# zhoubin-me/agent0

Measured on NVIDIA B200. Metric: replay_sample_target_transitions_per_sec, higher is better.
Workload: dtype u8 frames / f32 targets / f64 n-step returns

## Files before the change

### agent0_b200/_lib.py

```python
import ctypes as C
import os

import torch

_PKG = os.path.dirname(os.path.abspath(__file__))
LIB_PATH = os.environ.get("A0_LIB") or os.path.join(_PKG, "libagent0_b200.so")

A0_SLOTS = 8
A0_REC_META_I32 = 14
A0_MAX_NSTEP = 16
A0_MAX_ACTIONS = 32
A0_MAX_QUANTILES = 256
PTR_FRAMES, PTR_REC_SLOTS, PTR_REC_INFO, PTR_TREE, PTR_MAX_P = range(5)
OPT_PDL = 1
K2B_PLAN_MAX = 1024
K2B_PLAN_BYTES = 90176


def lz4_stride(frame_bytes):
    n = 8 * int(frame_bytes)
    return (n + n // 255 + 20 + 15) // 16 * 16

_vp, _i32, _i64, _f32, _f64 = C.c_void_p, C.c_int32, C.c_int64, C.c_float, C.c_double


class LossCommon(C.Structure):
    _fields_ = [("B", _i32), ("A", _i32), ("action", _vp), ("reward", _vp), ("done", _vp),
                ("weight", _vp), ("gamma_n", _f32), ("alpha", _f32), ("eps", _f32),
                ("loss", _vp), ("prio", _vp), ("max_p", _vp)]


class Plan(C.Structure):
    _fields_ = [("m", _i32), ("n_new", _i32), ("n_marks", _i32), ("new_frame_pos", C.POINTER(_i32)),
                ("rec_meta", C.POINTER(_i32)), ("marks", C.POINTER(_i32))]


class Merge(C.Structure):
    _fields_ = [("n_place", _i64), ("place", C.POINTER(_i64)), ("n_rec", _i64), ("record_map", C.POINTER(_i64)),
                ("n_tail", _i64), ("tails", C.POINTER(_i64)), ("stride_hint", _i64)]


IX_HEAD_Q, IX_TAIL_Q, IX_HEAD_FS, IX_TOP, IX_REC_CAPACITY, IX_FRAME_CAPACITY, IX_NSTEP, IX_AGE_LIMIT, \
    IX_MAX_CHUNK, IX_STATE_WORDS = range(10)
INGEST_FRAMES_ON_DEVICE, INGEST_FRAMES_PINNED, INGEST_COPY_STREAM = 1, 2, 4

SIGNATURES = {
    "a0_version": (_i32, []),
    "a0_last_error": (C.c_char_p, []),
    "a0_set_option": (_i32, [_i32, _i64]),
    "a0_get_option": (_i32, [_i32, C.POINTER(C.c_int64)]),
    "a0_rb_create": (_i32, [C.POINTER(_vp), _i64, _i64, _i32, _i32]),
    "a0_rb_destroy": (_i32, [_vp]),
    "a0_rb_reset": (_i32, [_vp, _vp]),
    "a0_rb_ptr": (_vp, [_vp, _i32]),
    "a0_rb_tree_leaves": (_i64, [_vp]),
    "a0_ix_create": (_i32, [C.POINTER(_vp), _i64, _i64, _i32, _i64]),
    "a0_ix_destroy": (_i32, [_vp]),
    "a0_ix_state": (_i32, [_vp, _vp]),
    "a0_ix_sampleable": (_vp, [_vp]),
    "a0_ix_set_stack": (_i32, [_vp, _i64, _vp]),
    "a0_ix_get_stack": (_i32, [_vp, _i64, _vp]),
    "a0_ix_resolve_shift": (_i32, [_vp, _vp, _vp, _i32, _vp]),
    "a0_ix_plan": (_i32, [_vp, _vp, _vp, _i32, _i32, _vp, _vp, _vp, C.POINTER(Plan)]),
    "a0_dd_create": (_i32, [C.POINTER(_vp), _i32]),
    "a0_dd_destroy": (_i32, [_vp]),
    "a0_dd_resolve": (_i32, [_vp, _vp, _vp, _vp, _i32, _vp, _vp, C.POINTER(_i32)]),
    "a0_ex_create": (_i32, [C.POINTER(_vp), _vp, _vp]),
    "a0_ex_destroy": (_i32, [_vp]),
    "a0_ex_extend": (_i32, [_vp, _vp, _vp, _vp, _vp, _vp, _vp, _i32, _f32, _vp]),
    "a0_ex_extend_v": (_i32, [_vp, _vp, _vp, _vp, _vp, _vp, _vp, _i32, _f32, _vp]),
    "a0_ex_decode": (_i32, [_vp, _vp, _vp, _i32, _vp, _vp, _vp]),
    "a0_ex_resolve": (_i32, [_vp, _vp, _vp, _i32, _vp, _vp, C.POINTER(_i32)]),
    "a0_ex_last_timing": (_i32, [_vp, _vp]),
    "a0_lz4_encode": (_i32, [_vp, _i32, _i32, _vp, _vp, _vp, _vp]),
    "a0_ix_serialize": (_i32, [_vp, _vp, _i64, C.POINTER(_i64)]),
    "a0_ix_deserialize": (_i32, [_vp, _vp, _i64]),
    "a0_ckpt_save": (_i32, [_vp, _vp, _vp, C.c_char_p, _vp, _i64, _vp]),
    "a0_ckpt_load": (_i32, [_vp, _vp, _vp, C.c_char_p, _vp, _i64, C.POINTER(_i64), _vp]),
    "a0_ckpt_last_timing": (_i32, [_vp]),
    "a0_ix_merge": (_i32, [_vp, _i32, _vp, _vp, _vp, _vp, _vp, _vp, _vp, _vp, _vp, _vp, _vp, C.POINTER(Merge)]),
    "a0_ckpt_info": (_i32, [C.c_char_p, _vp, _vp, _i64]),
    "a0_ckpt_merge": (_i32, [_vp, _vp, _vp, _vp, _i32, _vp, _vp, _vp, _vp, _i64, _vp, _vp]),
    "a0_rb_ingest_plan": (_i32, [_vp, C.POINTER(Plan), _vp, _vp, _i32, _f32, _vp]),
    "a0_rb_ingest_steps": (_i32, [_vp, _vp, _vp, _vp, _vp, _i32, _vp, _vp, _vp, _i32, _f32, _vp]),
    "a0_rb_ingest_steps_dyn": (_i32, [_vp, _vp, _vp, _vp, _vp, _i32, _vp, _vp, _vp, _i32, _f32, _f32, _i32, _vp]),
    "a0_rb_append": (_i32, [_vp, _vp, _vp, _i32, _vp, _i32, _vp]),
    "a0_pt_mark": (_i32, [_vp, _vp, _i32, _f32, _vp]),
    "a0_pt_update": (_i32, [_vp, _vp, _vp, _i32, _f32, _f32, _vp]),
    "a0_pt_update_report": (_i32, [_vp, _vp, _vp, _i32, _f32, _f32, _vp, _vp, _vp]),
    "a0_pt_update_overlapped": (_i32, [_vp, _vp, _vp, _i32, _f32, _f32, _vp, _vp, _vp]),
    "a0_pt_update_plan": (_i32, [_vp, _vp, _i32, _vp, _vp]),
    "a0_pt_update_apply": (_i32, [_vp, _vp, _vp, _i32, _f32, _f32, _vp, _vp, _vp, _vp]),
    "a0_host_map": (_i32, [_vp, C.POINTER(_vp)]),
    "a0_pt_set": (_i32, [_vp, _vp, _vp, _i32, _vp]),
    "a0_rb_set_dynamic": (_i32, [_vp, _f32, _f32, _f32, _vp]),
    "a0_pt_sample": (_i32, [_vp, _vp, _i32, _i32, _f32, _f32, _f32, _i32, _vp, _vp, _vp, _vp]),
    "a0_pt_sample_rng": (_i32, [_vp, C.c_uint64, _i64, _i32, _i32, _f32, _f32, _f32, _i32, _vp, _vp, _vp, _vp, _vp]),
    "a0_pt_rng_seek": (_i32, [_vp, C.c_uint64, _vp]),
    "a0_pt_sample_unique": (_i32, [_vp, C.c_uint64, _i64, _i32, _i32, _f32, _f32, _f32, _i32, _vp, _vp, _vp, _vp, _vp]),
    "a0_rb_gather": (_i32, [_vp, _vp, _i32, _i32, _f64, _vp, _vp, _vp, _vp, _vp, _vp, _vp, _i32, _vp]),
    "a0_rb_sample_gather": (_i32, [_vp, _vp, C.c_uint64, _i64, _i32, _i32, _f32, _f32, _f32, _i32, _vp, _vp, _vp, _i32, _f64,
                                   _vp, _vp, _vp, _vp, _vp, _vp, _vp, _vp]),
    "a0_rb_sample_mail": (_i32, [_vp, _vp, C.c_uint64, _i64, _i32, _i32, _f32, _f32, _f32, _i32, _vp, _vp, _vp, _vp]),
    "a0_rb_gather_mail": (_i32, [_vp, _i32, _i32, _i32, _i32, _f64, _vp, _vp, _vp, _vp, _vp, _vp, _vp, _vp]),
    "a0_rb_gather_unpaired": (_i32, [_vp, _i32, _vp, _vp]),
    "a0_rb_check_fault": (_i32, [_vp]),
    "a0_rb_gather_f32": (_i32, [_vp, _vp, _i32, _i32, _f64, _vp, _vp, _i32, _vp, _vp, _vp, _vp, _vp, _vp, _vp]),
    "a0_rb_gather_bf16": (_i32, [_vp, _vp, _i32, _i32, _f64, _vp, _vp, _i32, _vp, _vp, _vp, _vp, _vp, _vp, _vp]),
    "a0_loss_dqn": (_i32, [C.POINTER(LossCommon), _vp, _vp, _vp, _vp, _vp]),
    "a0_loss_mdqn": (_i32, [C.POINTER(LossCommon), _vp, _vp, _vp, _f32, _f32, _vp, _vp]),
    "a0_loss_c51": (_i32, [C.POINTER(LossCommon), _vp, _vp, _vp, _vp, _i32, _f32, _f32, _vp, _vp, _vp]),
    "a0_loss_quantile": (_i32, [C.POINTER(LossCommon), _i32, _vp, _vp, _vp, _vp, _i32, _i32, _vp,
                                _vp, _vp, _vp, _vp, _vp]),
    "a0_act_epsilon_greedy": (_i32, [_vp, _i32, _i32, _f64, _vp, _vp, _vp, _vp, _vp, _vp, _vp]),
    "a0_u8_to_f32": (_i32, [_vp, _vp, _i64, _i32, _vp]),
}

_lib = None


def load():
    global _lib
    if _lib is not None:
        return _lib
    if not os.path.exists(LIB_PATH):
        raise RuntimeError(
            f"{LIB_PATH} is missing: build it with `python -m agent0_b200.build` "
            "(agent0_b200 has no CPU fallback)")
    lib = C.CDLL(LIB_PATH)
    for name, (res, args) in SIGNATURES.items():
        fn = getattr(lib, name)
        fn.restype, fn.argtypes = res, args
    _lib = lib
    return lib


_pyingest = False


def pyingest():
    global _pyingest
    if _pyingest is False:
        path = os.path.join(_PKG, "_a0_pyingest.so")
        _pyingest = None
        if os.path.exists(path):
            try:
                h = C.PyDLL(path)
                h.a0_py_unpack.restype = _i64
                h.a0_py_unpack.argtypes = [C.py_object, _i64, _vp, _vp, _vp, _vp, _vp, _vp]
                h.a0_py_release.restype = None
                h.a0_py_release.argtypes = [_i64, _vp]
                h.a0_py_buffer_size.restype = _i64
                _pyingest = h
            except OSError:
                _pyingest = None
    return _pyingest


def check(rc, what):
    if rc != 0:
        msg = load().a0_last_error().decode(errors="replace")
        raise RuntimeError(f"{what} failed (code {rc}): {msg}")


_raw_stream = getattr(torch._C, "_cuda_getCurrentRawStream", None)


def stream_ptr(device=None):
    if _raw_stream is not None:
        if device is None:
            idx = torch.cuda.current_device()
        elif isinstance(device, int):
            idx = device
        else:
            idx = device.index if device.index is not None else torch.cuda.current_device()
        return _raw_stream(idx)
    return torch.cuda.current_stream(device).cuda_stream


def ptr(t, dtype=None):
    if t is None:
        return None
    if not t.is_cuda:
        raise RuntimeError("agent0_b200 kernels need CUDA tensors (there is no CPU path)")
    if dtype is not None and t.dtype != dtype:
        raise TypeError(f"expected {dtype}, got {t.dtype}")
    if not t.is_contiguous():
        raise ValueError("tensor must be contiguous")
    return t.data_ptr()


def host_map(t):
    if t.is_cuda or not t.is_pinned():
        raise ValueError("host_map needs a pinned CPU tensor")
    out = _vp()
    check(load().a0_host_map(t.data_ptr(), C.byref(out)), "a0_host_map")
    return out.value


class HandleOwner:

    def __init__(self, lib, handle):
        self.lib, self.handle = lib, handle

    def __del__(self):
        try:
            if self.handle is not None and self.handle.value:
                self.lib.a0_rb_destroy(self.handle)
                self.handle = None
        except Exception:
            pass


class _DevView:

    def __init__(self, address, shape, typestr, owner=None):
        self.owner = owner
        self.__cuda_array_interface__ = {"shape": tuple(shape), "typestr": typestr,
                                         "data": (int(address), False), "version": 2}


def device_view(address, shape, typestr, device, owner=None):
    return torch.as_tensor(_DevView(address, shape, typestr, owner), device=device)
```

### agent0_b200/csrc/a0_targets.cu

```cuda
#include <stdlib.h>

#include "a0_common.cuh"
#ifdef A0_TRACE
A0_TRACE_SETTER(a0_trace_set_targets)
#endif

struct A0Common {
  int32_t B, A;
  const int64_t* action;
  const float* reward;
  const float* done;
  const float* weight;
  float gamma_n, alpha, eps;
  float* loss;
  float* prio;
  float* max_p;
};

static inline A0Common a0_unpack(const a0_loss_common_t* c) {
  A0Common k;
  k.B = c->B; k.A = c->A; k.action = c->action; k.reward = c->reward; k.done = c->done;
  k.weight = c->weight; k.gamma_n = c->gamma_n; k.alpha = c->alpha; k.eps = c->eps;
  k.loss = c->loss; k.prio = c->prio; k.max_p = c->max_p;
  return k;
// ... 174 lines not shown
    if (!spec) l[k] = in ? orow[lane + 32 * k] : -INFINITY;
    s_m[wid][lane + 32 * k] = 0.0f;
  }
  if (spec) {
#pragma unroll
    for (int a2 = 0; a2 < C51_SPEC_A; ++a2)
      if (a2 == a) { l[0] = lo_all[a2][0]; l[1] = lo_all[a2][1]; }
  }

  float omx = -INFINITY;
#pragma unroll
  for (int k = 0; k < C51_MAXR; ++k) omx = fmaxf(omx, l[k]);
#ifdef A0_TRACE
  if (omx == 12345.678f) printf("x");
#endif
  A0_TX(0);
  int a_star;
  if (qsel) {
    float v = qs;
    int vi = lane;
#pragma unroll
    for (int o = 16; o > 0; o >>= 1) {
      const float ov = __shfl_xor_sync(0xffffffffu, v, o);
      const int oi = __shfl_xor_sync(0xffffffffu, vi, o);
      const float om = __shfl_xor_sync(0xffffffffu, omx, o);
      if (ov > v || (ov == v && oi < vi)) { v = ov; vi = oi; }
      omx = fmaxf(omx, om);
    }
    a_star = vi;
  } else {
    omx = a0_warp_max(omx);
    float best = -INFINITY;
    a_star = 0;
    for (int a2 = 0; a2 < A; ++a2) {
      const float* row = tgt_logits + ((size_t)b * A + a2) * M;
      float v[C51_MAXR], mx = -INFINITY;
#pragma unroll
      for (int k = 0; k < C51_MAXR; ++k) {
        v[k] = (k < R && lane + 32 * k < M) ? row[lane + 32 * k] : -INFINITY;
        mx = fmaxf(mx, v[k]);
      }
      mx = a0_warp_max(mx);
      float se = 0.0f;
#pragma unroll
      for (int k = 0; k < C51_MAXR; ++k) { v[k] = (k < R && lane + 32 * k < M) ? expf(v[k] - mx) : 0.0f; se += v[k]; }
      se = a0_warp_sum(se);
      float ev = 0.0f;
#pragma unroll
      for (int k = 0; k < C51_MAXR; ++k) ev += __fdiv_rn(v[k], se) * z[k];
      ev = a0_warp_sum(ev);
      if (ev > best) { best = ev; a_star = a2; }
    }
  }

  A0_TX(1);
  const float* trow = tgt_logits + ((size_t)b * A + a_star) * M;
  float p[C51_MAXR], mx = -INFINITY;
#pragma unroll
  for (int k = 0; k < C51_MAXR; ++k) p[k] = -INFINITY;
  if (spec) {
#pragma unroll
    for (int a2 = 0; a2 < C51_SPEC_A; ++a2)
      if (a2 == a_star) { p[0] = tg_all[a2][0]; p[1] = tg_all[a2][1]; }
  } else {
#pragma unroll
    for (int k = 0; k < C51_MAXR; ++k)
      if (k < R && lane + 32 * k < M) p[k] = trow[lane + 32 * k];
  }
#pragma unroll
  for (int k = 0; k < C51_MAXR; ++k) mx = fmaxf(mx, p[k]);
  float ose = 0.0f;
#pragma unroll
  for (int k = 0; k < C51_MAXR; ++k) ose += (k < R && lane + 32 * k < M) ? expf(l[k] - omx) : 0.0f;
#pragma unroll
  for (int o = 16; o > 0; o >>= 1) {
    const float om = __shfl_xor_sync(0xffffffffu, mx, o);
    const float os = __shfl_xor_sync(0xffffffffu, ose, o);
    mx = fmaxf(mx, om);
    ose += os;
  }
  float se = 0.0f;
#pragma unroll
  for (int k = 0; k < C51_MAXR; ++k) { p[k] = (k < R && lane + 32 * k < M) ? expf(p[k] - mx) : 0.0f; se += p[k]; }
  se = a0_warp_sum(se);

  A0_TX(2);
  const float gm = __fmul_rn(c.gamma_n, __fsub_rn(1.0f, d));
  const float delta = (vmax - vmin) / (float)(M - 1);
  int lo[C51_MAXR], up[C51_MAXR];
  float wlo[C51_MAXR], wup[C51_MAXR];
#pragma unroll
  for (int k = 0; k < C51_MAXR; ++k) {
    lo[k] = up[k] = -1;
    wlo[k] = wup[k] = 0.0f;
    if (k < R && lane + 32 * k < M) {
      const float pj = __fdiv_rn(p[k], se);
      float tz = __fadd_rn(r, __fmul_rn(gm, z[k]));
      tz = fminf(fmaxf(tz, vmin), vmax);
      const float base = __fdiv_rn(__fsub_rn(tz, vmin), delta);
      int lo_ = (int)floorf(base), up_ = (int)ceilf(base);
      if (up_ > 0 && lo_ == up_) lo_ -= 1;
      if (lo_ < M - 1 && lo_ == up_) up_ += 1;
      lo[k] = lo_; up[k] = up_ < M ? up_ : -1;
      wlo[k] = __fmul_rn(pj, __fsub_rn((float)up_, base));
      wup[k] = __fmul_rn(pj, __fsub_rn(base, (float)lo_));
    }
  }
  __syncwarp();
  A0_TX(3);
  if (R <= 2) {
    const int key4[4] = {lo[0], lo[1], up[0], up[1]};
    float val4[4] = {wlo[0], wlo[1], wup[0], wup[1]};
    a0_c51_scatter<4>(s_m[wid], key4, val4, lane);
  } else {
    a0_c51_scatter<C51_MAXR>(s_m[wid], lo, wlo, lane);
    a0_c51_scatter<C51_MAXR>(s_m[wid], up, wup, lane);
  }
  float m[C51_MAXR];
#pragma unroll
  for (int k = 0; k < C51_MAXR; ++k) m[k] = s_m[wid][lane + 32 * k];

  A0_TX(4);
  const float lse = logf(ose);
  float ce = 0.0f, msum = 0.0f;
#pragma unroll
  for (int k = 0; k < C51_MAXR; ++k)
    if (k < R && lane + 32 * k < M) { ce += m[k] * ((l[k] - omx) - lse); msum += m[k]; }
  ce = a0_warp_sum(ce);
  msum = a0_warp_sum(msum);
  A0_TX(5);
  float* grow = grad + (size_t)b * A * M;
  for (int a2 = 0; a2 < A; ++a2) {
    if (a2 == a) continue;
    for (int j = lane; j < M; j += 32) grow[(size_t)a2 * M + j] = 0.0f;
  }
#pragma unroll
  for (int k = 0; k < C51_MAXR; ++k) {
    const int j = lane + 32 * k;
    if (k < R && j < M) {
      const float sm = expf((l[k] - omx) - lse);
      grow[(size_t)a * M + j] = w * (sm * msum - m[k]);
      if (target_prob) target_prob[(size_t)b * M + j] = m[k];
    }
  }
  A0_TX(6);
  if (lane == 0) a0_emit(c, b, -ce);
  A0_TX(7);
#ifdef A0_TRACE
  _t2 = _t2 * 0 + (unsigned long long)_c0;
#endif
  if (threadIdx.x == 0) A0_TEND(4);
}

template <int WARPS>
__global__ void __launch_bounds__(WARPS * 32)
a0_k4_c51_fast(const A0Common c, const float* __restrict__ logits, const float* __restrict__ tgt_logits,
               const float* __restrict__ qsel, const float* __restrict__ atoms, int32_t M, float vmin, float vmax,
               float delta, float* __restrict__ grad, float* __restrict__ target_prob) {
  __shared__ float s_m[WARPS][72];
  A0_T0();
  A0_PDL_PROLOGUE();
  A0_TMID();
#ifdef A0_TRACE
  const long long _c0 = clock64();
#endif
  const int lane = threadIdx.x & 31;
  const int wid = threadIdx.x >> 5;
  const int b = blockIdx.x * WARPS + wid;
  if (b >= c.B) return;
  const int A = c.A;
  const bool in0 = lane < M, in1 = lane + 32 < M;
  float lo_all[C51_SPEC_A][2], tg_all[C51_SPEC_A][2], qs[C51_SPEC_A];
  const float* lrow = logits + (size_t)b * A * M + lane;
  const float* trow = tgt_logits + (size_t)b * A * M + lane;
  const float* qrow = qsel + (size_t)b * A;
#pragma unroll
  for (int a2 = 0; a2 < C51_SPEC_A; ++a2) {
    const bool on = a2 < A;
    lo_all[a2][0] = (on && in0) ? lrow[a2 * M] : -INFINITY;
    lo_all[a2][1] = (on && in1) ? lrow[a2 * M + 32] : -INFINITY;
    tg_all[a2][0] = (on && in0) ? trow[a2 * M] : -INFINITY;
    tg_all[a2][1] = (on && in1) ? trow[a2 * M + 32] : -INFINITY;
    qs[a2] = on ? qrow[a2] : -INFINITY;
  }
  const int a = (int)c.action[b];
  const float r = c.reward[b], d = c.done[b], w = c.weight[b];
  const float z0 = in0 ? atoms[lane] : 0.0f, z1 = in1 ? atoms[lane + 32] : 0.0f;
  s_m[wid][lane] = 0.0f;
  s_m[wid][lane + 32] = 0.0f;
  const int AM = A * M, r0 = a * M;
  float* gb = grad + (size_t)b * AM;
  for (int e = lane; e < AM; e += 32)
    if (e < r0 || e >= r0 + M) gb[e] = 0.0f;
  int a_star = 0;
  float best = qs[0];
#pragma unroll
  for (int a2 = 1; a2 < C51_SPEC_A; ++a2)
    if (qs[a2] > best) { best = qs[a2]; a_star = a2; }
  float l0 = -INFINITY, l1 = -INFINITY, p0 = -INFINITY, p1 = -INFINITY;
#pragma unroll
  for (int a2 = 0; a2 < C51_SPEC_A; ++a2) {
    if (a2 == a) { l0 = lo_all[a2][0]; l1 = lo_all[a2][1]; }
    if (a2 == a_star) { p0 = tg_all[a2][0]; p1 = tg_all[a2][1]; }
  }
  A0_TX(0);
  float omx = fmaxf(l0, l1), mx = fmaxf(p0, p1);
#pragma unroll
  for (int o = 16; o > 0; o >>= 1) {
    const float a_ = __shfl_xor_sync(0xffffffffu, omx, o);
    const float b_ = __shfl_xor_sync(0xffffffffu, mx, o);
    omx = fmaxf(omx, a_);
    mx = fmaxf(mx, b_);
  }
  A0_TX(1);
  const float eo0 = in0 ? expf(l0 - omx) : 0.0f, eo1 = in1 ? expf(l1 - omx) : 0.0f;
  p0 = in0 ? expf(p0 - mx) : 0.0f;
  p1 = in1 ? expf(p1 - mx) : 0.0f;
  float ose = eo0 + eo1, se = p0 + p1;
#pragma unroll
  for (int o = 16; o > 0; o >>= 1) {
    const float a_ = __shfl_xor_sync(0xffffffffu, ose, o);
    const float b_ = __shfl_xor_sync(0xffffffffu, se, o);
    ose += a_;
    se += b_;
  }
  A0_TX(2);
  const float gm = __fmul_rn(c.gamma_n, __fsub_rn(1.0f, d));
  int k0 = -1, k1 = -1;
  float wl0 = 0.0f, wu0 = 0.0f, wl1 = 0.0f, wu1 = 0.0f;
  {
    const float pj0 = p0 != 0.0f ? __fdiv_rn(p0, se) : 0.0f, pj1 = p1 != 0.0f ? __fdiv_rn(p1, se) : 0.0f;
    const float tz0 = fminf(fmaxf(__fadd_rn(r, __fmul_rn(gm, z0)), vmin), vmax);
    const float tz1 = fminf(fmaxf(__fadd_rn(r, __fmul_rn(gm, z1)), vmin), vmax);
    const float nu0 = __fsub_rn(tz0, vmin), nu1 = __fsub_rn(tz1, vmin);
    const float bs0 = nu0 != 0.0f ? __fdiv_rn(nu0, delta) : 0.0f, bs1 = nu1 != 0.0f ? __fdiv_rn(nu1, delta) : 0.0f;
    const int c0 = max((int)ceilf(bs0) - 1, 0), c1 = max((int)ceilf(bs1) - 1, 0);
    if (in0) { k0 = c0; wl0 = __fmul_rn(pj0, __fsub_rn((float)(c0 + 1), bs0)); wu0 = __fmul_rn(pj0, __fsub_rn(bs0, (float)c0)); }
    if (in1) { k1 = c1; wl1 = __fmul_rn(pj1, __fsub_rn((float)(c1 + 1), bs1)); wu1 = __fmul_rn(pj1, __fsub_rn(bs1, (float)c1)); }
  }
  A0_TX(3);
#pragma unroll
  for (int dd = 1; dd < 32; dd <<= 1) {
    const int q0 = __shfl_up_sync(0xffffffffu, k0, dd), q1 = __shfl_up_sync(0xffffffffu, k1, dd);
    const float a0_ = __shfl_up_sync(0xffffffffu, wl0, dd), b0_ = __shfl_up_sync(0xffffffffu, wu0, dd);
    const float a1_ = __shfl_up_sync(0xffffffffu, wl1, dd), b1_ = __shfl_up_sync(0xffffffffu, wu1, dd);
    if (lane >= dd && q0 == k0) { wl0 = __fadd_rn(wl0, a0_); wu0 = __fadd_rn(wu0, b0_); }
    if (lane >= dd && q1 == k1) { wl1 = __fadd_rn(wl1, a1_); wu1 = __fadd_rn(wu1, b1_); }
  }
  const int n0 = __shfl_down_sync(0xffffffffu, k0, 1), n1 = __shfl_down_sync(0xffffffffu, k1, 1);
  const bool tail0 = k0 >= 0 && (lane == 31 || n0 != k0), tail1 = k1 >= 0 && (lane == 31 || n1 != k1);
  float* bins = s_m[wid];
  __syncwarp();
  if (tail0) bins[k0] = __fadd_rn(bins[k0], wl0);
  __syncwarp();
  if (tail1) bins[k1] = __fadd_rn(bins[k1], wl1);
  __syncwarp();
  if (tail0) bins[k0 + 1] = __fadd_rn(bins[k0 + 1], wu0);
  __syncwarp();
  if (tail1) bins[k1 + 1] = __fadd_rn(bins[k1 + 1], wu1);
  __syncwarp();
  const float m0 = bins[lane], m1 = bins[lane + 32];
  A0_TX(4);
  const float lse = logf(ose);
  const float ls0 = (l0 - omx) - lse, ls1 = (l1 - omx) - lse;
  float ce = 0.0f, msum = 0.0f;
  if (in0) { ce += m0 * ls0; msum += m0; }
  if (in1) { ce += m1 * ls1; msum += m1; }
#pragma unroll
  for (int o = 16; o > 0; o >>= 1) {
    const float a_ = __shfl_xor_sync(0xffffffffu, ce, o);
    const float b_ = __shfl_xor_sync(0xffffffffu, msum, o);
    ce += a_;
    msum += b_;
  }
  A0_TX(5);
  if (lane == 0) a0_emit(c, b, -ce);
  const float g0 = w * (expf(ls0) * msum - m0), g1 = w * (expf(ls1) * msum - m1);
  if (in0) gb[r0 + lane] = g0;
  if (in1) gb[r0 + lane + 32] = g1;
  if (target_prob) {
    if (in0) target_prob[(size_t)b * M + lane] = m0;
    if (in1) target_prob[(size_t)b * M + lane + 32] = m1;
  }
  A0_TX(6);
  A0_TX(7);
#ifdef A0_TRACE
  _t2 = _t2 * 0 + (unsigned long long)_c0;
#endif
  if (threadIdx.x == 0) A0_TEND(4);
}

static int g_c51_fast = -1;
static bool a0_option_c51_fast() {
  if (g_c51_fast < 0) {
    const char* e = getenv("A0_C51_FAST");
    g_c51_fast = e ? (atoi(e) != 0) : 1;
  }
  return g_c51_fast != 0;
}
void a0_set_c51_fast(int on) { g_c51_fast = on != 0; }

extern "C" int a0_loss_c51(const a0_loss_common_t* c, const float* logits, const float* tgt_logits,
                           const float* qsel, const float* atoms, int32_t M, float vmin, float vmax, float* grad,
                           float* target_prob, a0_stream_t stream) {
  int rc = a0_check_common(c, "a0_loss_c51");
  if (rc) return rc;
  A0_REQUIRE(logits && tgt_logits && atoms && grad, "a0_loss_c51: NULL tensor");
  A0_REQUIRE(M >= 2 && M <= C51_MAXR * 32, "a0_loss_c51: num_atoms %d outside [2,%d]", M, C51_MAXR * 32);
  A0_REQUIRE(vmax > vmin, "a0_loss_c51: vmax must exceed vmin");
  if (c->B == 0) return A0_OK;
  if (qsel && c->A <= C51_SPEC_A && M <= 64 && a0_option_c51_fast()) {
    const float delta = (vmax - vmin) / (float)(M - 1);
    static int warps = 0;
    if (!warps) {
      const char* e = getenv("A0_C51_WARPS");
      warps = e ? atoi(e) : C51_FAST_WARPS;
      if (warps != 1 && warps != 2 && warps != 4 && warps != 8 && warps != 16 && warps != 32) warps = C51_FAST_WARPS;
    }
    const unsigned grid = (unsigned)((c->B + warps - 1) / warps);
#define A0_C51_FAST_LAUNCH(W)                                                                                              \
    A0_LAUNCH(a0_k4_c51_fast<W>, grid, W * 32, 0, (cudaStream_t)stream, 1, A0_PDL_K4, a0_unpack(c), logits, tgt_logits, qsel,   \
              atoms, M, vmin, vmax, delta, grad, target_prob)
    if (warps == 1) A0_C51_FAST_LAUNCH(1);
    else if (warps == 2) A0_C51_FAST_LAUNCH(2);
    else if (warps == 4) A0_C51_FAST_LAUNCH(4);
    else if (warps == 8) A0_C51_FAST_LAUNCH(8);
    else if (warps == 16) A0_C51_FAST_LAUNCH(16);
    else A0_C51_FAST_LAUNCH(32);
#undef A0_C51_FAST_LAUNCH
    return A0_OK;
  }
  A0_LAUNCH(a0_k4_c51, (unsigned)((c->B + C51_WARPS - 1) / C51_WARPS), C51_WARPS * 32, 0, (cudaStream_t)stream, 1, A0_PDL_K4,
            a0_unpack(c), logits, tgt_logits, qsel, atoms, M, vmin, vmax, grad, target_prob);
  return A0_OK;
}

constexpr int QH_SPEC_A = 8;

__device__ __forceinline__ float a0_block_sum(float v, float* red, int nwarps) {
  v = a0_warp_sum(v);
  __syncthreads();
  if ((threadIdx.x & 31) == 0) red[threadIdx.x >> 5] = v;
  __syncthreads();
  float s = 0.0f;
  for (int i = 0; i < nwarps; ++i) s += red[i];
  return s;
}

template <bool SPEC>
__global__ void __launch_bounds__(A0_MAX_QUANTILES)
a0_k4_quantile(const A0Common c, int32_t layout, const float* __restrict__ q, const float* __restrict__ qt,
               const float* __restrict__ taus, const float* __restrict__ qsel, int32_t Ni, int32_t Nj,
               float* __restrict__ grad, const float* __restrict__ q_bar, const float* __restrict__ taus_full,
               float* __restrict__ fraction_loss, float* __restrict__ grad_taus) {
  __shared__ float sT[A0_MAX_QUANTILES];
  __shared__ float sQ[A0_MAX_QUANTILES];
  __shared__ float sMean[A0_MAX_ACTIONS];
  __shared__ float red[A0_MAX_QUANTILES / 32];
  __shared__ int s_astar;
  A0_PDL_PROLOGUE();
  const int b = blockIdx.x;
  const int tid = threadIdx.x, lane = tid & 31, wid = tid >> 5;
  const int nwarps = blockDim.x >> 5;
  const int A = c.A;
  const size_t sN_q = layout == 0 ? 1 : (size_t)A, sA_q = layout == 0 ? (size_t)Nj : 1;
  const size_t sN_t = layout == 0 ? 1 : (size_t)A, sA_t = layout == 0 ? (size_t)Ni : 1;
  const float* qb = q + (size_t)b * A * Nj;
  const float* tb = qt + (size_t)b * A * Ni;

  float qj = 0.0f, tau = 0.0f, w;
  int a;
  if (SPEC) {
    a = (int)c.action[b];
    const float r = c.reward[b], d = c.done[b];
    w = c.weight[b];
    float qs[QH_SPEC_A], tv[QH_SPEC_A], qv[QH_SPEC_A];
#pragma unroll
    for (int a2 = 0; a2 < QH_SPEC_A; ++a2) {
      const bool on = a2 < A;
      qs[a2] = on ? qsel[(size_t)b * A + a2] : -INFINITY;
      tv[a2] = (on && tid < Ni) ? tb[(size_t)tid * A + a2] : 0.0f;
      qv[a2] = (on && tid < Nj) ? qb[(size_t)tid * A + a2] : 0.0f;
    }
    if (tid < Nj) tau = taus[(size_t)b * Nj + tid];
    int a_star = 0;
    float best = qs[0];
#pragma unroll
    for (int a2 = 1; a2 < QH_SPEC_A; ++a2)
      if (qs[a2] > best) { best = qs[a2]; a_star = a2; }
    float tsel = 0.0f;
#pragma unroll
    for (int a2 = 0; a2 < QH_SPEC_A; ++a2) {
      if (a2 == a_star) tsel = tv[a2];
      if (a2 == a) qj = qv[a2];
    }
    if (tid < Ni) sT[tid] = a0_td_target(r, d, c.gamma_n, tsel);
    if (tid < Nj) sQ[tid] = qj;
    __syncthreads();
  } else {
  if (qsel) {
    if (wid == 0) {
      const int as = a0_warp_argmax(lane < A ? qsel[(size_t)b * A + lane] : -INFINITY, lane);
      if (lane == 0) s_astar = as;
    }
  } else {
    for (int a2 = wid; a2 < A; a2 += nwarps) {
      float s = 0.0f;
      for (int i = lane; i < Ni; i += 32) s += tb[a2 * sA_t + i * sN_t];
      s = a0_warp_sum(s);
      if (lane == 0) sMean[a2] = __fdiv_rn(s, (float)Ni);
    }
    __syncthreads();
    if (wid == 0) {
      const int as = a0_warp_argmax(lane < A ? sMean[lane] : -INFINITY, lane);
      if (lane == 0) s_astar = as;
    }
  }
  __syncthreads();
  const int a_star = s_astar;
  a = (int)c.action[b];
  const float r = c.reward[b], d = c.done[b];
  w = c.weight[b];
  if (tid < Ni) sT[tid] = a0_td_target(r, d, c.gamma_n, tb[a_star * sA_t + tid * sN_t]);
  if (tid < Nj) {
    qj = qb[a * sA_q + tid * sN_q];
    tau = taus ? taus[(size_t)b * Nj + tid] : __fdiv_rn((float)(2 * tid + 1), 2.0f * (float)Nj);
    sQ[tid] = qj;
  }
  __syncthreads();
  }

  float lsum = 0.0f, gsum = 0.0f;
  if (tid < Nj) {
    float lp = 0.0f, ln = 0.0f, gp = 0.0f, gn = 0.0f;
#pragma unroll 8
    for (int i = 0; i < Ni; ++i) {
      const float uij = qj - sT[i];
      const float a_ = fabsf(uij);
      const float c_ = fminf(a_, 1.0f);
      const float x_ = fmaf(-0.5f, c_, a_);
      if (uij > 0.0f) { lp = fmaf(c_, x_, lp); gp += c_; }
      else { ln = fmaf(c_, x_, ln); gn += c_; }
    }
    const float k_pos = 1.0f - tau;
    lsum = fmaf(k_pos, lp, tau * ln);
    gsum = fmaf(k_pos, gp, -tau * gn);
  }
  const float total = a0_block_sum(lsum, red, nwarps);
  float* gb = grad + (size_t)b * A * Nj;
  for (int i = tid; i < A * Nj; i += blockDim.x) gb[i] = 0.0f;
  __syncthreads();
  if (tid < Nj) gb[a * sA_q + tid * sN_q] = __fdiv_rn(w, (float)Ni) * gsum;
  if (tid == 0) a0_emit(c, b, __fdiv_rn(total, (float)Ni));

  if (q_bar) {
    const int F = Nj;
    float gi = 0.0f, contrib = 0.0f;
    if (tid < F - 1) {
      const float* qbar_b = q_bar + (size_t)b * (F - 1) * A;
      const float qi = qbar_b[(size_t)tid * A + a];
      const float prev = tid == 0 ? sQ[0] : qbar_b[(size_t)(tid - 1) * A + a];
      const float next = tid == F - 2 ? sQ[F - 1] : qbar_b[(size_t)(tid + 1) * A + a];
      const float v1 = qi - sQ[tid], v2 = qi - sQ[tid + 1];
      gi = (qi > prev ? v1 : -v1) + (qi < next ? v2 : -v2);
      contrib = gi * taus_full[(size_t)b * (F + 1) + tid + 1];
    }
    const float fl = a0_block_sum(contrib, red, nwarps);
    if (tid == 0 && fraction_loss) fraction_loss[b] = fl;
    if (grad_taus) {
      float* gt = grad_taus + (size_t)b * (F + 1);
      if (tid < F - 1) gt[tid + 1] = w * gi;
      if (tid == 0) { gt[0] = 0.0f; gt[F] = 0.0f; }
    }
  }
}

constexpr int QS_MAX = A0_MAX_QUANTILES;
static_assert(QS_MAX == 256, "the merge tree below is written for 8 runs of 32");

__device__ __forceinline__ float a0_qs_next_up(float x) {
  const uint32_t b = __float_as_uint(x);
  if (x == 0.0f) return __uint_as_float(1u);
  return __uint_as_float((b >> 31) ? b - 1u : b + 1u);
}
__device__ __forceinline__ float a0_qs_pad(int idx) { return __uint_as_float(0x7f7fff00u + (uint32_t)idx); }

// ... 461 lines not shown
```

### include/agent0_b200.h

```cpp
#ifndef AGENT0_B200_H
#define AGENT0_B200_H

#include <stddef.h>
#include <stdint.h>

#ifdef __cplusplus
extern "C" {
#endif

typedef struct a0_replay a0_replay_t;
typedef struct a0_index a0_index_t;
typedef void* a0_stream_t;

#define A0_OK 0
#define A0_EINVAL (-1)
#define A0_ENOMEM (-2)
#define A0_EFAULT (-3)
#define A0_STACK 4
#define A0_SLOTS 8
#define A0_MAX_NSTEP 16
#define A0_MAX_ACTIONS 32
#define A0_MAX_QUANTILES 256
#define A0_REC_META_I32 14

// ... 57 lines not shown
int a0_dd_resolve(a0_dedupe_t* dd, a0_index_t* ix, const int64_t* stream, const uint8_t* frames,
                  int32_t m, int64_t* fs8_out, int64_t* new_src_out, int32_t* n_new_out);

typedef struct a0_extend a0_extend_t;
int a0_ex_create(a0_extend_t** out, a0_replay_t* h, a0_index_t* ix);
int a0_ex_destroy(a0_extend_t* ex);
int a0_ex_extend(a0_extend_t* ex, const uint8_t* blobs , const int64_t* blob_len ,
                 const int64_t* stream, const int64_t* action, const double* reward, const uint8_t* done,
                 int32_t m, float alpha, a0_stream_t cuda_stream);
int a0_ex_extend_v(a0_extend_t* ex, const uint8_t* const* blob_ptr ,
                   const int64_t* blob_len , const int64_t* stream, const int64_t* action,
                   const double* reward, const uint8_t* done, int32_t m, float alpha,
                   a0_stream_t cuda_stream);
int a0_ex_decode(a0_extend_t* ex, const uint8_t* blobs , const int64_t* blob_len ,
                 int32_t m, uint8_t* frames_out , int32_t* status_out ,
                 a0_stream_t cuda_stream);
int a0_ex_resolve(a0_extend_t* ex, const int64_t* stream, const uint8_t* labels, int32_t m,
                  int64_t* fs8_out, int64_t* new_src_out, int32_t* n_new_out);
int a0_ex_last_timing(a0_extend_t* ex, float* out6);

#define A0_LZ4_STRIDE(frame_bytes) \
  ((((int64_t)8 * (frame_bytes) + (int64_t)8 * (frame_bytes) / 255 + 20) + 15) / 16 * 16)
int a0_lz4_encode(const uint8_t* frames , int32_t m, int32_t frame_bytes, uint8_t* out ,
                  int32_t* out_len , uint64_t* frame_hash , a0_stream_t stream);

int a0_ix_serialize(a0_index_t* ix, uint8_t* out, int64_t cap, int64_t* len_out);
int a0_ix_deserialize(a0_index_t* ix, const uint8_t* blob, int64_t len);
int a0_ckpt_save(a0_replay_t* h, a0_index_t* ix, a0_extend_t* ex, const char* path, const uint8_t* user,
                 int64_t user_len, a0_stream_t stream);
int a0_ckpt_load(a0_replay_t* h, a0_index_t* ix, a0_extend_t* ex, const char* path, uint8_t* user_out,
                 int64_t user_cap, int64_t* user_len_out, a0_stream_t stream);
int a0_ckpt_last_timing(double* out8);

typedef struct {
  int64_t n_place;
  const int64_t* place;
  int64_t n_rec;
  const int64_t* record_map;
  int64_t n_tail;
  const int64_t* tails;
  int64_t stride_hint;
} a0_merge_t;
int a0_ix_merge(a0_index_t* target, int32_t k, a0_index_t* const* src, const uint8_t* const* records,
                const float* const* leaves, const int64_t* map_old, const int64_t* map_new, const int64_t* map_len,
                const int64_t* tail_count, const int64_t* tail_ids, const int64_t* tail_seq, uint8_t* records_out,
                float* leaves_out, a0_merge_t* out);
int a0_ckpt_info(const char* path, int64_t* out8, int64_t* ids_out, int64_t ids_cap);
int a0_ckpt_merge(a0_replay_t* h, a0_index_t* ix, a0_extend_t* ex, const char* const* paths, int32_t k,
                  const int64_t* map_old, const int64_t* map_new, const int64_t* map_len, uint8_t* user_out,
                  int64_t user_cap, int64_t* user_len_out, a0_stream_t stream);

#define A0_INGEST_FRAMES_ON_DEVICE 1
#define A0_INGEST_FRAMES_PINNED 2
#define A0_INGEST_COPY_STREAM 4
int a0_rb_ingest_plan(a0_replay_t* h, const a0_plan_t* plan, const uint8_t* frames,
                      const int64_t* new_frame_src, int32_t flags, float alpha, a0_stream_t stream);
int a0_rb_ingest_steps(a0_replay_t* h, a0_index_t* ix, const int64_t* stream, const int64_t* n_new,
                       const uint8_t* new_frames, int32_t flags, const int64_t* action,
                       const double* reward, const uint8_t* done, int32_t m, float alpha,
                       a0_stream_t cuda_stream);
int a0_rb_ingest_steps_dyn(a0_replay_t* h, a0_index_t* ix, const int64_t* stream,
                           const int64_t* n_new, const uint8_t* new_frames, int32_t flags,
                           const int64_t* action, const double* reward, const uint8_t* done,
                           int32_t m, float alpha, float beta, int32_t compat_sum,
                           a0_stream_t cuda_stream);

int a0_pt_mark(a0_replay_t* h, const int32_t* pos , int32_t count, float alpha,
               a0_stream_t stream);
int a0_pt_update(a0_replay_t* h, const int64_t* idx , const float* loss ,
                 int32_t count, float alpha, float eps, a0_stream_t stream);
int a0_pt_set(a0_replay_t* h, const int64_t* idx , const float* value ,
              int32_t count, a0_stream_t stream);
int a0_pt_update_report(a0_replay_t* h, const int64_t* idx , const float* loss ,
                        int32_t count, float alpha, float eps, int64_t* idx_report ,
                        float* loss_report , a0_stream_t stream);
int a0_pt_update_overlapped(a0_replay_t* h, const int64_t* idx , const float* loss ,
                            int32_t count, float alpha, float eps, int64_t* idx_report, float* loss_report,
                            a0_stream_t stream);
#define A0_K2B_PLAN_MAX 1024
#define A0_K2B_PLAN_BYTES 90176
int a0_pt_update_plan(a0_replay_t* h, const int64_t* idx , int32_t count, void* plan ,
                      a0_stream_t stream);
int a0_pt_update_apply(a0_replay_t* h, const int64_t* idx , const float* loss , int32_t count,
                       float alpha, float eps, const void* plan , int64_t* idx_report, float* loss_report,
                       a0_stream_t stream);
int a0_host_map(const void* host_ptr, void** dev_ptr_out);

int a0_rb_set_dynamic(a0_replay_t* h, float top, float beta, float sum_offset, a0_stream_t stream);
int a0_pt_sample(a0_replay_t* h, const float* u , int32_t total, int32_t batch,
                 float top, float beta, float sum_offset, int32_t uniform,
                 int64_t* idx_out , float* prio_out ,
                 float* weight_out , a0_stream_t stream);

int a0_pt_sample_rng(a0_replay_t* h, uint64_t seed, int64_t call, int32_t total, int32_t batch,
                     float top, float beta, float sum_offset, int32_t uniform, int64_t* idx_out,
                     float* prio_out, float* weight_out, float* u_out, a0_stream_t stream);
int a0_pt_rng_seek(a0_replay_t* h, uint64_t call, a0_stream_t stream);

int a0_pt_sample_unique(a0_replay_t* h, uint64_t seed, int64_t call, int32_t total, int32_t batch,
                        float top, float beta, float sum_offset, int32_t uniform, int64_t* idx_out,
                        float* prio_out, float* weight_out, int32_t* stats_out, a0_stream_t stream);

int a0_rb_gather(a0_replay_t* h, const int64_t* idx , int32_t count, int32_t n_step,
                 double gamma, uint8_t* frames_out, int64_t* action_out, double* reward64_out,
                 float* reward32_out, uint8_t* done8_out, float* done32_out, int64_t* boot_out,
                 int32_t variant, a0_stream_t stream);

int a0_rb_sample_gather(a0_replay_t* h, const float* u , uint64_t seed,
                        int64_t call, int32_t total, int32_t batch, float top, float beta,
                        float sum_offset, int32_t uniform, int64_t* idx_out, float* prio_out,
                        float* weight_out, int32_t n_step, double gamma, uint8_t* frames_out,
                        int64_t* action_out, double* reward64_out, float* reward32_out,
                        uint8_t* done8_out, float* done32_out, int64_t* boot_out, a0_stream_t stream);

int a0_rb_sample_mail(a0_replay_t* h, const float* u , uint64_t seed, int64_t call,
                      int32_t total, int32_t batch, float top, float beta, float sum_offset, int32_t uniform,
                      int64_t* idx_out, float* prio_out, float* weight_out, a0_stream_t stream);
int a0_rb_gather_mail(a0_replay_t* h, int32_t lo, int32_t count, int32_t window, int32_t n_step, double gamma,
                      uint8_t* frames_out, int64_t* action_out, double* reward64_out, float* reward32_out,
                      uint8_t* done8_out, float* done32_out, int64_t* boot_out, a0_stream_t stream);

int a0_rb_gather_unpaired(a0_replay_t* h, int32_t count, uint8_t* frames_out, a0_stream_t stream);
int a0_rb_check_fault(a0_replay_t* h);

int a0_rb_gather_f32(a0_replay_t* h, const int64_t* idx , int32_t count, int32_t n_step,
                     double gamma, float* obs_out, float* next_out, int32_t norm_mode,
                     int64_t* action_out, double* reward64_out, float* reward32_out,
                     uint8_t* done8_out, float* done32_out, int64_t* boot_out, a0_stream_t stream);
int a0_rb_gather_bf16(a0_replay_t* h, const int64_t* idx , int32_t count, int32_t n_step,
                      double gamma, uint16_t* obs_out, uint16_t* next_out, int32_t norm_mode,
                      int64_t* action_out, double* reward64_out, float* reward32_out,
                      uint8_t* done8_out, float* done32_out, int64_t* boot_out, a0_stream_t stream);

typedef struct {
  int32_t B, A;
  const int64_t* action;
  const float* reward;
  const float* done;
  const float* weight;
  float gamma_n;
  float alpha, eps;
  float* loss;
  float* prio;
  float* max_p;
} a0_loss_common_t;

int a0_loss_dqn(const a0_loss_common_t* c, const float* q, const float* qt_next, const float* qsel,
                float* grad, a0_stream_t stream);
int a0_loss_mdqn(const a0_loss_common_t* c, const float* q, const float* qt_next,
                 const float* qt_cur, float tau, float lo, float* grad, a0_stream_t stream);
int a0_loss_c51(const a0_loss_common_t* c, const float* logits, const float* tgt_logits,
                const float* qsel, const float* atoms, int32_t M, float vmin, float vmax,
                float* grad, float* target_prob, a0_stream_t stream);
int a0_loss_quantile(const a0_loss_common_t* c, int32_t layout, const float* q, const float* qt,
                     const float* taus, const float* qsel, int32_t Ni, int32_t Nj, float* grad,
                     const float* q_bar, const float* taus_full, float* fraction_loss,
                     float* grad_taus, a0_stream_t stream);

int a0_act_epsilon_greedy(const float* q , int32_t E, int32_t A, double epsilon,
                          const double* u , const int64_t* action_random ,
                          int64_t* action_out, float* qmax_out, float* scratch, float* qmax_mean,
                          a0_stream_t stream);
int a0_u8_to_f32(const uint8_t* in , float* out , int64_t count, int32_t norm_mode,
                 a0_stream_t stream);

#ifdef __cplusplus
}
#endif
#endif
```

Baseline: 10.30 million.

## Restructure C51 fast kernel projection with reciprocal division and conflict-free bin scatter

In the fast C51 target kernel, the fp32 division by delta becomes a double-precision reciprocal multiply with one FMA correction. A check kernel is added to verify it bit-exactly against __fdiv_rn. The warp max reductions use redux.sync, and the segmented-scan join masks are computed once, earlier, and overlapped with the sum reduction. The four serialized shared-memory read-modify-write bin updates become writes into four separate term arrays that are summed afterwards, and softmax exponentials are hoisted. This shortens the serial dependency chain at the cost of more shared memory and fp64 ops, and redux.sync.f32 needs recent hardware.

```diff
diff --git a/agent0_b200/_lib.py b/agent0_b200/_lib.py
--- a/agent0_b200/_lib.py
+++ b/agent0_b200/_lib.py
@@ -110,6 +110,7 @@
     "a0_loss_dqn": (_i32, [C.POINTER(LossCommon), _vp, _vp, _vp, _vp, _vp]),
     "a0_loss_mdqn": (_i32, [C.POINTER(LossCommon), _vp, _vp, _vp, _f32, _f32, _vp, _vp]),
     "a0_loss_c51": (_i32, [C.POINTER(LossCommon), _vp, _vp, _vp, _vp, _i32, _f32, _f32, _vp, _vp, _vp]),
+    "a0_c51_div_check": (_i32, [_f32, _f32, _i32, _vp, _vp]),
     "a0_loss_quantile": (_i32, [C.POINTER(LossCommon), _i32, _vp, _vp, _vp, _vp, _i32, _i32, _vp,
                                 _vp, _vp, _vp, _vp, _vp]),
     "a0_act_epsilon_greedy": (_i32, [_vp, _i32, _i32, _f64, _vp, _vp, _vp, _vp, _vp, _vp, _vp]),
diff --git a/agent0_b200/csrc/a0_targets.cu b/agent0_b200/csrc/a0_targets.cu
--- a/agent0_b200/csrc/a0_targets.cu
+++ b/agent0_b200/csrc/a0_targets.cu
@@ -350,12 +350,30 @@
   if (threadIdx.x == 0) A0_TEND(4);
 }
 
+
+__device__ __forceinline__ float a0_warp_max_redux(float v) {
+  float m;
+  asm("redux.sync.max.f32 %0, %1, 0xffffffff;" : "=f"(m) : "f"(v));
+  return m;
+}
+
+__device__ __forceinline__ float a0_c51_div_delta(float nu, float delta, double rdelta) {
+  const double q0 = __dmul_rn((double)nu, rdelta);
+  const double rem = __fma_rn(-q0, (double)delta, (double)nu);
+  return __double2float_rn(__fma_rn(rem, rdelta, q0));
+}
+
+static void a0_c51_delta(float vmin, float vmax, int32_t M, float* delta, double* rdelta) {
+  *delta = (vmax - vmin) / (float)(M - 1);
+  *rdelta = 1.0 / (double)*delta;
+}
+
 template <int WARPS>
 __global__ void __launch_bounds__(WARPS * 32)
 a0_k4_c51_fast(const A0Common c, const float* __restrict__ logits, const float* __restrict__ tgt_logits,
                const float* __restrict__ qsel, const float* __restrict__ atoms, int32_t M, float vmin, float vmax,
-               float delta, float* __restrict__ grad, float* __restrict__ target_prob) {
-  __shared__ float s_m[WARPS][72];
+               float delta, double rdelta, float* __restrict__ grad, float* __restrict__ target_prob) {
+  __shared__ float s_t[WARPS][4][72];
   A0_T0();
   A0_PDL_PROLOGUE();
   A0_TMID();
@@ -384,8 +402,12 @@
   const int a = (int)c.action[b];
   const float r = c.reward[b], d = c.done[b], w = c.weight[b];
   const float z0 = in0 ? atoms[lane] : 0.0f, z1 = in1 ? atoms[lane + 32] : 0.0f;
-  s_m[wid][lane] = 0.0f;
-  s_m[wid][lane + 32] = 0.0f;
+  float(*terms)[72] = s_t[wid];
+#pragma unroll
+  for (int t = 0; t < 4; ++t) {
+    terms[t][lane] = 0.0f;
+    terms[t][lane + 32] = 0.0f;
+  }
   const int AM = A * M, r0 = a * M;
   float* gb = grad + (size_t)b * AM;
   for (int e = lane; e < AM; e += 32)
@@ -402,19 +424,30 @@
     if (a2 == a_star) { p0 = tg_all[a2][0]; p1 = tg_all[a2][1]; }
   }
   A0_TX(0);
-  float omx = fmaxf(l0, l1), mx = fmaxf(p0, p1);
-#pragma unroll
-  for (int o = 16; o > 0; o >>= 1) {
-    const float a_ = __shfl_xor_sync(0xffffffffu, omx, o);
-    const float b_ = __shfl_xor_sync(0xffffffffu, mx, o);
-    omx = fmaxf(omx, a_);
-    mx = fmaxf(mx, b_);
-  }
+  const float omx = a0_warp_max_redux(fmaxf(l0, l1)), mx = a0_warp_max_redux(fmaxf(p0, p1));
   A0_TX(1);
-  const float eo0 = in0 ? expf(l0 - omx) : 0.0f, eo1 = in1 ? expf(l1 - omx) : 0.0f;
-  p0 = in0 ? expf(p0 - mx) : 0.0f;
-  p1 = in1 ? expf(p1 - mx) : 0.0f;
+  const float eo0 = expf(in0 ? l0 - omx : -INFINITY), eo1 = expf(in1 ? l1 - omx : -INFINITY);
+  p0 = expf(in0 ? p0 - mx : -INFINITY);
+  p1 = expf(in1 ? p1 - mx : -INFINITY);
   float ose = eo0 + eo1, se = p0 + p1;
+  const float gm = __fmul_rn(c.gamma_n, __fsub_rn(1.0f, d));
+  const float tz0 = fminf(fmaxf(__fadd_rn(r, __fmul_rn(gm, z0)), vmin), vmax);
+  const float tz1 = fminf(fmaxf(__fadd_rn(r, __fmul_rn(gm, z1)), vmin), vmax);
+  const float bs0 = a0_c51_div_delta(__fsub_rn(tz0, vmin), delta, rdelta);
+  const float bs1 = a0_c51_div_delta(__fsub_rn(tz1, vmin), delta, rdelta);
+  const int c0 = max((int)ceilf(bs0) - 1, 0), c1 = max((int)ceilf(bs1) - 1, 0);
+  const int k0 = in0 ? c0 : -1, k1 = in1 ? c1 : -1;
+  const float fl0 = __fsub_rn((float)(c0 + 1), bs0), fu0 = __fsub_rn(bs0, (float)c0);
+  const float fl1 = __fsub_rn((float)(c1 + 1), bs1), fu1 = __fsub_rn(bs1, (float)c1);
+  unsigned join0 = 0, join1 = 0;
+#pragma unroll
+  for (int s = 0; s < 5; ++s) {
+    const int q0 = __shfl_up_sync(0xffffffffu, k0, 1 << s), q1 = __shfl_up_sync(0xffffffffu, k1, 1 << s);
+    if (lane >= (1 << s) && q0 == k0) join0 |= 1u << s;
+    if (lane >= (1 << s) && q1 == k1) join1 |= 1u << s;
+  }
+  const int n0 = __shfl_down_sync(0xffffffffu, k0, 1), n1 = __shfl_down_sync(0xffffffffu, k1, 1);
+  const bool tail0 = k0 >= 0 && (lane == 31 || n0 != k0), tail1 = k1 >= 0 && (lane == 31 || n1 != k1);
 #pragma unroll
   for (int o = 16; o > 0; o >>= 1) {
     const float a_ = __shfl_xor_sync(0xffffffffu, ose, o);
@@ -422,45 +455,34 @@
     ose += a_;
     se += b_;
   }
+  const float lse = logf(ose);
+  const float ls0 = (l0 - omx) - lse, ls1 = (l1 - omx) - lse;
+  float sm0 = expf(ls0), sm1 = expf(ls1);
   A0_TX(2);
-  const float gm = __fmul_rn(c.gamma_n, __fsub_rn(1.0f, d));
-  int k0 = -1, k1 = -1;
   float wl0 = 0.0f, wu0 = 0.0f, wl1 = 0.0f, wu1 = 0.0f;
   {
-    const float pj0 = p0 != 0.0f ? __fdiv_rn(p0, se) : 0.0f, pj1 = p1 != 0.0f ? __fdiv_rn(p1, se) : 0.0f;
-    const float tz0 = fminf(fmaxf(__fadd_rn(r, __fmul_rn(gm, z0)), vmin), vmax);
-    const float tz1 = fminf(fmaxf(__fadd_rn(r, __fmul_rn(gm, z1)), vmin), vmax);
-    const float nu0 = __fsub_rn(tz0, vmin), nu1 = __fsub_rn(tz1, vmin);
-    const float bs0 = nu0 != 0.0f ? __fdiv_rn(nu0, delta) : 0.0f, bs1 = nu1 != 0.0f ? __fdiv_rn(nu1, delta) : 0.0f;
-    const int c0 = max((int)ceilf(bs0) - 1, 0), c1 = max((int)ceilf(bs1) - 1, 0);
-    if (in0) { k0 = c0; wl0 = __fmul_rn(pj0, __fsub_rn((float)(c0 + 1), bs0)); wu0 = __fmul_rn(pj0, __fsub_rn(bs0, (float)c0)); }
-    if (in1) { k1 = c1; wl1 = __fmul_rn(pj1, __fsub_rn((float)(c1 + 1), bs1)); wu1 = __fmul_rn(pj1, __fsub_rn(bs1, (float)c1)); }
+    const float q0 = __fdiv_rn(p0 != 0.0f ? p0 : 1.0f, se), q1 = __fdiv_rn(p1 != 0.0f ? p1 : 1.0f, se);
+    const float pj0 = p0 != 0.0f ? q0 : 0.0f, pj1 = p1 != 0.0f ? q1 : 0.0f;
+    if (in0) { wl0 = __fmul_rn(pj0, fl0); wu0 = __fmul_rn(pj0, fu0); }
+    if (in1) { wl1 = __fmul_rn(pj1, fl1); wu1 = __fmul_rn(pj1, fu1); }
   }
   A0_TX(3);
 #pragma unroll
-  for (int dd = 1; dd < 32; dd <<= 1) {
-    const int q0 = __shfl_up_sync(0xffffffffu, k0, dd), q1 = __shfl_up_sync(0xffffffffu, k1, dd);
-    const float a0_ = __shfl_up_sync(0xffffffffu, wl0, dd), b0_ = __shfl_up_sync(0xffffffffu, wu0, dd);
-    const float a1_ = __shfl_up_sync(0xffffffffu, wl1, dd), b1_ = __shfl_up_sync(0xffffffffu, wu1, dd);
-    if (lane >= dd && q0 == k0) { wl0 = __fadd_rn(wl0, a0_); wu0 = __fadd_rn(wu0, b0_); }
-    if (lane >= dd && q1 == k1) { wl1 = __fadd_rn(wl1, a1_); wu1 = __fadd_rn(wu1, b1_); }
-  }
-  const int n0 = __shfl_down_sync(0xffffffffu, k0, 1), n1 = __shfl_down_sync(0xffffffffu, k1, 1);
-  const bool tail0 = k0 >= 0 && (lane == 31 || n0 != k0), tail1 = k1 >= 0 && (lane == 31 || n1 != k1);
-  float* bins = s_m[wid];
+  for (int s = 0; s < 5; ++s) {
+    const float a0_ = __shfl_up_sync(0xffffffffu, wl0, 1 << s), b0_ = __shfl_up_sync(0xffffffffu, wu0, 1 << s);
+    const float a1_ = __shfl_up_sync(0xffffffffu, wl1, 1 << s), b1_ = __shfl_up_sync(0xffffffffu, wu1, 1 << s);
+    if (join0 >> s & 1u) { wl0 = __fadd_rn(wl0, a0_); wu0 = __fadd_rn(wu0, b0_); }
+    if (join1 >> s & 1u) { wl1 = __fadd_rn(wl1, a1_); wu1 = __fadd_rn(wu1, b1_); }
+  }
+  asm volatile("" : "+f"(sm0), "+f"(sm1));
   __syncwarp();
-  if (tail0) bins[k0] = __fadd_rn(bins[k0], wl0);
+  if (tail0) { terms[0][k0] = wl0; terms[2][k0 + 1] = wu0; }
+  if (tail1) { terms[1][k1] = wl1; terms[3][k1 + 1] = wu1; }
   __syncwarp();
-  if (tail1) bins[k1] = __fadd_rn(bins[k1], wl1);
-  __syncwarp();
-  if (tail0) bins[k0 + 1] = __fadd_rn(bins[k0 + 1], wu0);
-  __syncwarp();
-  if (tail1) bins[k1 + 1] = __fadd_rn(bins[k1 + 1], wu1);
-  __syncwarp();
-  const float m0 = bins[lane], m1 = bins[lane + 32];
+  const float m0 = __fadd_rn(__fadd_rn(__fadd_rn(terms[0][lane], terms[1][lane]), terms[2][lane]), terms[3][lane]);
+  const float m1 = __fadd_rn(__fadd_rn(__fadd_rn(terms[0][lane + 32], terms[1][lane + 32]), terms[2][lane + 32]),
+                             terms[3][lane + 32]);
   A0_TX(4);
-  const float lse = logf(ose);
-  const float ls0 = (l0 - omx) - lse, ls1 = (l1 - omx) - lse;
   float ce = 0.0f, msum = 0.0f;
   if (in0) { ce += m0 * ls0; msum += m0; }
   if (in1) { ce += m1 * ls1; msum += m1; }
@@ -473,7 +495,7 @@
   }
   A0_TX(5);
   if (lane == 0) a0_emit(c, b, -ce);
-  const float g0 = w * (expf(ls0) * msum - m0), g1 = w * (expf(ls1) * msum - m1);
+  const float g0 = w * (sm0 * msum - m0), g1 = w * (sm1 * msum - m1);
   if (in0) gb[r0 + lane] = g0;
   if (in1) gb[r0 + lane + 32] = g1;
   if (target_prob) {
@@ -507,8 +529,10 @@
   A0_REQUIRE(M >= 2 && M <= C51_MAXR * 32, "a0_loss_c51: num_atoms %d outside [2,%d]", M, C51_MAXR * 32);
   A0_REQUIRE(vmax > vmin, "a0_loss_c51: vmax must exceed vmin");
   if (c->B == 0) return A0_OK;
-  if (qsel && c->A <= C51_SPEC_A && M <= 64 && a0_option_c51_fast()) {
-    const float delta = (vmax - vmin) / (float)(M - 1);
+  float delta;
+  double rdelta;
+  a0_c51_delta(vmin, vmax, M, &delta, &rdelta);
+  if (qsel && c->A <= C51_SPEC_A && M <= 64 && delta > 0.0f && delta < INFINITY && a0_option_c51_fast()) {
     static int warps = 0;
     if (!warps) {
       const char* e = getenv("A0_C51_WARPS");
@@ -518,7 +542,7 @@
     const unsigned grid = (unsigned)((c->B + warps - 1) / warps);
 #define A0_C51_FAST_LAUNCH(W)                                                                                              \
     A0_LAUNCH(a0_k4_c51_fast<W>, grid, W * 32, 0, (cudaStream_t)stream, 1, A0_PDL_K4, a0_unpack(c), logits, tgt_logits, qsel,   \
-              atoms, M, vmin, vmax, delta, grad, target_prob)
+              atoms, M, vmin, vmax, delta, rdelta, grad, target_prob)
     if (warps == 1) A0_C51_FAST_LAUNCH(1);
     else if (warps == 2) A0_C51_FAST_LAUNCH(2);
     else if (warps == 4) A0_C51_FAST_LAUNCH(4);
@@ -530,6 +554,38 @@
   }
   A0_LAUNCH(a0_k4_c51, (unsigned)((c->B + C51_WARPS - 1) / C51_WARPS), C51_WARPS * 32, 0, (cudaStream_t)stream, 1, A0_PDL_K4,
             a0_unpack(c), logits, tgt_logits, qsel, atoms, M, vmin, vmax, grad, target_prob);
+  return A0_OK;
+}
+
+__global__ void a0_c51_div_check_kernel(uint32_t hi, float delta, double rdelta, unsigned long long* out) {
+  unsigned long long bad = 0, first = ~0ull;
+  for (unsigned long long u = blockIdx.x * (unsigned long long)blockDim.x + threadIdx.x; u <= hi;
+       u += (unsigned long long)gridDim.x * blockDim.x) {
+    const float nu = __uint_as_float((uint32_t)u);
+    if (__float_as_uint(a0_c51_div_delta(nu, delta, rdelta)) != __float_as_uint(__fdiv_rn(nu, delta))) {
+      ++bad;
+      first = min(first, u);
+    }
+  }
+  if (bad) {
+    atomicAdd(out, bad);
+    atomicMin(out + 1, first);
+  }
+}
+
+extern "C" int a0_c51_div_check(float vmin, float vmax, int32_t M, unsigned long long* out, a0_stream_t stream) {
+  A0_REQUIRE(out != nullptr, "a0_c51_div_check: NULL output");
+  A0_REQUIRE(M >= 2 && vmax > vmin, "a0_c51_div_check: M %d, vmin %g, vmax %g", M, (double)vmin, (double)vmax);
+  float delta;
+  double rdelta;
+  a0_c51_delta(vmin, vmax, M, &delta, &rdelta);
+  A0_REQUIRE(delta > 0.0f && delta < INFINITY, "a0_c51_div_check: delta %g is zero or infinite", (double)delta);
+  const float hi = vmax - vmin;
+  A0_REQUIRE(hi < INFINITY, "a0_c51_div_check: vmax - vmin overflows");
+  uint32_t hb;
+  memcpy(&hb, &hi, sizeof(hb));
+  a0_c51_div_check_kernel<<<148 * 8, 256, 0, (cudaStream_t)stream>>>(hb, delta, rdelta, out);
+  A0_LAUNCH_CHECK();
   return A0_OK;
 }
 
diff --git a/include/agent0_b200.h b/include/agent0_b200.h
--- a/include/agent0_b200.h
+++ b/include/agent0_b200.h
@@ -233,6 +233,7 @@
 int a0_loss_c51(const a0_loss_common_t* c, const float* logits, const float* tgt_logits,
                 const float* qsel, const float* atoms, int32_t M, float vmin, float vmax,
                 float* grad, float* target_prob, a0_stream_t stream);
+int a0_c51_div_check(float vmin, float vmax, int32_t M, unsigned long long* out, a0_stream_t stream);
 int a0_loss_quantile(const a0_loss_common_t* c, int32_t layout, const float* q, const float* qt,
                      const float* taus, const float* qsel, int32_t Ni, int32_t Nj, float* grad,
                      const float* q_bar, const float* taus_full, float* fraction_loss,
```

Measured after the change: 11.51 million, median of 6. 1.12x the previous value.
